# lucasnewman/f5-tts-mlx

Hardware: AMD Instinct MI355X
Metric: mel_frames_per_sec (higher is better)
Workload: dtype f16 (IEEE-half MFMA operands, fp32 accumulate / residual stream / LayerNorm / softmax state; meets the 1e-3 gate); 1 GPU; BASELINE configs[1]: F5-TTS 335M, 32-point euler (=62 DiT forwards, CFG), batch 1/GPU x 10 s (N=937) utterances, hipGraph=True; f16 (IEEE half) MFMA operands IN PLACE OF BASELINE's bf16 -- same width and MFMA rate, three more significand bits; plain bf16 fails the 1e-3 parity gate, see sub.b1_bf16; global_batch=1, seq_len=937, parallelism=dp1 (utterance sharding)

## Files before the change

### f5_tts_mlx_amd/csrc/convpos.hpp

```cpp
#include "op16.hpp"

#if F5_F16
#ifndef F5_CONVPOS_HPP_F16
#define F5_CONVPOS_HPP_F16
#define F5_CONVPOS_HPP_BODY
#endif
#else
#ifndef F5_CONVPOS_HPP_BF16
#define F5_CONVPOS_HPP_BF16
#define F5_CONVPOS_HPP_BODY
#endif
#endif
#ifdef F5_CONVPOS_HPP_BODY
#undef F5_CONVPOS_HPP_BODY
namespace F5_NS {

struct F5ConvPosArgs {
    const op16_t* in[2];
    const op16_t* W[2];
    const float* bias;
    int B, seq_len, C, groups, taps, ld;
    int nseg;
    int mode;
    op16_t* out_bf[2];
    float* out_f32;
    int ldo;
    int* sat_flag;
};

int f5_launch_convpos(const F5ConvPosArgs& a, hipStream_t stream);
}
#endif
```

### f5_tts_mlx_amd/csrc/engine.hip

```cpp
#include <stdarg.h>

#include <string>
#include <vector>

#include "../../include/f5tts_hip.h"
#include "host_common.hpp"

static Ops g_ops;

static thread_local char g_err[1024] = "";
void f5_set_error(const char* fmt, ...) {
    va_list ap;
    va_start(ap, fmt);
    vsnprintf(g_err, sizeof(g_err), fmt, ap);
    va_end(ap);
}
extern "C" const char* f5_last_error(void) { return g_err; }
extern "C" int f5_version(void) { return 1; }

struct MatF8 {
    size_t q = 0, s = 0;
    int rows = 0, ld = 0;
};
struct BlockW {
// ... 12 lines not shown
    size_t status;
    size_t lncnt, lncnt_words;
    size_t lens, dur2, text, ids, keep, rowkeep;
    size_t tgrid, dt, cfgv, sinus, th, temb, mod;
    size_t rope_cos, rope_sin;
    size_t rope_t;
    size_t cond, traj, ytmp, kst, vel;
    size_t xin[2];
    size_t te[2], tg, grn_partial, grn_nx;
    size_t tln[2], tg2[2], ct[2];
    size_t hc, x;
    size_t xb[2], c1[2], h[2], qk[2], vt[2], ao[2], ffh[2];
    size_t h8, h8s, ao8, ao8s, ffh8, ffh8s;
    size_t lnstats;
    size_t lnrowf;
    size_t lnmean;
    size_t foldc[2];
    bool fold_planned;
    size_t vt_bytes;
    size_t cond_keep;
};

struct F5Options {
    int q_premul = 1;
    int qkv_tr = 1;
    int fuse_ln = 0;
    int gemm_flags = 0;
    int attn_pipe = -1;
    int ln_fold = -1;
    int fold_stats = -1;
    int graph_split = 0;
    int sat_check = 1;
    int null_keeps_cond = 0;
};
static F5Options g_default_options;
static int g_live_engines = 0;
static int g_knob_epoch = 0;

struct f5_engine : WeightStore {
    f5_config cfg;
    int prec;
    size_t time_w0, time_b0, time_w2, time_b2;
    size_t ada_w, ada_b;
    size_t text_table, text_pos;
    std::vector<TextBlockW> tblocks;
    MatBF wx, wct;
    size_t bproj;
    MatBF conv_w[2];
    size_t conv_b[2];
    std::vector<BlockW> blocks;
    MatBF wout;
    size_t bout;
    Ops ops;
    F5Options opt = g_default_options;
    GraphCache graphs;
    std::vector<std::string> seen;
};

static int nfe_per_step(int method) { return method == F5_EULER ? 1 : (method == F5_MIDPOINT ? 2 : 4); }

static MatF8 alloc_f8(Bump& b, int rows, int ld) {
    MatF8 m;
    m.rows = rows;
    m.ld = ld;
    const int rows_pad = (rows + 255) / 256 * 256;
    m.q = b.take((size_t)rows_pad * ld);
// ... 123 lines not shown
    e->cfg = c;
    e->prec = precision;
    e->np = precision == F5_PREC_BF16X3 ? 2 : 1;
    e->f16 = e->ops.h = precision == F5_PREC_F16;
    build_arena_plan(e);
    ++g_live_engines;
    *out = e;
    return 0;
}

extern "C" void f5_engine_destroy(f5_engine* e) {
    if (!e) return;
    --g_live_engines;
    delete e;
}

extern "C" int f5_engine_set_graph_cache(f5_engine* e, int max_graphs) {
    F5_REQUIRE(e && max_graphs >= 1 && max_graphs <= 1024, "graph cache size must be in [1, 1024]");
    e->graphs.set_cap((size_t)max_graphs);
    return 0;
}

enum OptKind { OPT_SWITCH, OPT_TRI, OPT_INT };
static const struct OptDesc {
    const char* name;
    int F5Options::*member;
    OptKind kind;
} k_options[] = {
    {"q_premul", &F5Options::q_premul, OPT_SWITCH},     {"qkv_transposed", &F5Options::qkv_tr, OPT_SWITCH},
    {"ln_fusion", &F5Options::fuse_ln, OPT_SWITCH},     {"gemm_flags", &F5Options::gemm_flags, OPT_INT},
    {"attn_pipe", &F5Options::attn_pipe, OPT_TRI},      {"null_keeps_cond", &F5Options::null_keeps_cond, OPT_SWITCH},
    {"ln_fold", &F5Options::ln_fold, OPT_TRI},          {"sat_check", &F5Options::sat_check, OPT_SWITCH},
    {"graph_split", &F5Options::graph_split, OPT_SWITCH}, {"fold_stats", &F5Options::fold_stats, OPT_TRI},
};
static const OptDesc* find_option(const char* name) {
    std::string names;
    for (const OptDesc& o : k_options) {
        if (strcmp(o.name, name) == 0) return &o;
        names += names.empty() ? "" : ", ";
        names += o.name;
    }
    f5_set_error("unknown engine option %s (%s)", name, names.c_str());
    return nullptr;
}
extern "C" int f5_engine_set_option(f5_engine* e, const char* name, int value) {
    F5_REQUIRE(e && name, "null argument");
    const OptDesc* o = find_option(name);
    if (!o) return 2;
    e->opt.*o->member = o->kind == OPT_INT ? value : (o->kind == OPT_TRI && value < 0 ? -1 : (value ? 1 : 0));
    return 0;
}
extern "C" int f5_engine_get_option(f5_engine* e, const char* name, int* value) {
    F5_REQUIRE(e && name && value, "null argument");
    const OptDesc* o = find_option(name);
    if (!o) return 2;
    *value = e->opt.*o->member;
    return 0;
}
extern "C" int f5_engine_graph_count(f5_engine* e) { return e ? e->graphs.size() : -1; }

extern "C" int f5_weights_bytes(f5_engine* e, size_t* bytes) {
    F5_REQUIRE(e && bytes, "null argument");
    *bytes = e->arena_need;
    return 0;
}

extern "C" int f5_set_weights_arena(f5_engine* e, void* dev_arena, size_t bytes, void* stream) {
    F5_REQUIRE(e && dev_arena, "null argument");
    return e->set_arena(dev_arena, bytes, (hipStream_t)stream);
}

extern "C" int f5_load_tensor(f5_engine* e, const char* name, const float* host, int ndim, const int64_t* shape) {
    F5_REQUIRE(e && name && host && shape, "null argument");
    std::vector<TensorDst>* dsts = nullptr;
    size_t count = 0;
// ... 273 lines not shown
    int cur = 0;
    for (int i = 0; i < cf.conv_layers; ++i) {
        const TextBlockW& t = e->tblocks[i];
        RC(K.dwconv_ln(c.p<float>(w.te[cur]), c.a<float>(t.dw_w), c.a<float>(t.dw_b), c.a<float>(t.ln_w),
                               c.a<float>(t.ln_b), c.pb(w.tln, 0), c.pb(w.tln, 1), 2 * c.B, c.N, Dt, 1e-6f, s));
        F5GemmArgs g1 = gemm_base(c, c.pb(w.tln, 0), c.pb(w.tln, 1), Dt, t.pw1, M2, TF, Dt, c.a<float>(t.b1));
        g1.out_f32 = c.p<float>(w.tg);
        g1.ldo = TF;
        RC(K.gemm(g1, EPI_GELU_ERF, s));
        RC(K.grn(c.p<float>(w.tg), c.a<float>(t.gamma), c.a<float>(t.beta), c.p<float>(w.grn_partial),
                         c.p<float>(w.grn_nx), c.pb(w.tg2, 0), c.pb(w.tg2, 1), 2 * c.B, c.N, TF, s));
        F5GemmArgs g2 = gemm_base(c, c.pb(w.tg2, 0), c.pb(w.tg2, 1), TF, t.pw2, M2, Dt, TF, c.a<float>(t.b2));
        g2.out_f32 = c.p<float>(w.te[cur ^ 1]);
        g2.ldo = Dt;
        g2.resid = c.p<float>(w.te[cur]);
        g2.ldres = Dt;
        g2.rowkeep = c.p<uint8_t>(w.keep);
        RC(K.gemm(g2, EPI_RESID_KEEP, s));
        cur ^= 1;
    }
    if (c.edit)
        RC(K.pack_cond_text_keep(c.p<float>(w.cond), c.p<uint8_t>(w.cond_keep), c.p<float>(w.te[cur]), c.pb(w.ct, 0), c.pb(w.ct, 1),
                                 c.B, c.N, cf.mel_dim, Dt, e->opt.null_keeps_cond, s));
    else
        RC(K.pack_cond_text(c.p<float>(w.cond), c.p<int>(w.lens), c.p<float>(w.te[cur]), c.pb(w.ct, 0), c.pb(w.ct, 1), c.B,
                                c.N, cf.mel_dim, Dt, e->opt.null_keeps_cond, s));
    F5GemmArgs gh = gemm_base(c, c.pb(w.ct, 0), c.pb(w.ct, 1), 128 + Dt, e->wct, M2, D, 128 + Dt, c.a<float>(e->bproj));
    gh.out_f32 = c.p<float>(w.hc);
    gh.ldo = D;
    RC(K.gemm(gh, EPI_F32, s));
    return 0;
}

static int run_dit(const Ctx& c, int j) {
    const f5_engine* e = c.e;
    const f5_config& cf = e->cfg;
    const Workspace& w = c.w;
    const int D = cf.dim, FF = cf.ff_dim, L = cf.depth, H = cf.heads;
    const int M1 = c.B * c.N, M = c.nb * M1;
    hipStream_t s = c.s;
    const Ops& K = c.ops;
    const float* mod = c.p<float>(w.mod) + (size_t)j * (6 * L + 2) * D;
    const uint8_t* rowkeep = c.use_mask ? c.p<uint8_t>(w.rowkeep) : nullptr;
    const int* kvlen = c.use_mask ? c.p<int>(w.dur2) : nullptr;

    F5GemmArgs g0 = gemm_base(c, c.pb(w.xin, 0), c.pb(w.xin, 1), 128, e->wx, M, D, 128, nullptr);
    g0.a_row_mod = M1;
    g0.addrows = c.p<float>(w.hc);
    g0.ldadd = D;
    g0.out_f32 = c.p<float>(w.x);
    g0.ldo = D;
    g0.out_bf[0] = c.pb(w.xb, 0);
    g0.out_bf[1] = c.pb(w.xb, 1);
    g0.ldob = D;
    RC(K.gemm(g0, EPI_ADDROWS, s));

    F5ConvPosArgs cp;
    memset(&cp, 0, sizeof(cp));
    cp.B = c.nb * c.B;
    cp.seq_len = c.N;
    cp.C = D;
    cp.groups = cf.conv_pos_groups;
    cp.taps = cf.conv_pos_kernel;
    cp.ld = D;
    cp.ldo = D;
    cp.nseg = c.nseg();
    cp.in[0] = c.pb(w.xb, 0);
    cp.in[1] = c.pb(w.xb, 1);
    cp.W[0] = c.wm(e->conv_w[0], 0);
    cp.W[1] = c.wm(e->conv_w[0], 1);
    cp.bias = c.a<float>(e->conv_b[0]);
    cp.mode = 0;
    cp.out_bf[0] = c.pb(w.c1, 0);
    cp.out_bf[1] = c.pb(w.c1, 1);
    RC(K.convpos(cp, s));
    cp.in[0] = c.pb(w.c1, 0);
    cp.in[1] = c.pb(w.c1, 1);
    cp.W[0] = c.wm(e->conv_w[1], 0);
    cp.W[1] = c.wm(e->conv_w[1], 1);
    cp.bias = c.a<float>(e->conv_b[1]);
    cp.mode = 1;
    cp.out_bf[0] = cp.out_bf[1] = nullptr;
    cp.out_f32 = c.p<float>(w.x);
    RC(K.convpos(cp, s));

    const float qpre = q_premul_factor(e);
    for (int i = 0; i < L && e->prec == F5_PREC_MXFP8; ++i) {
        const BlockW& bw = e->blocks[i];
        const float* m6 = mod + (size_t)i * 6 * D;
        auto f8args = [&](const uint8_t* a8, const uint8_t* as, int lda, const MatF8& wm, int N_, int K_, const float* bias) {
            F5GemmArgs g;
            memset(&g, 0, sizeof(g));
            g.A8 = a8;
            g.As = as;
            g.lda8 = lda;
            g.W8 = (const uint8_t*)(e->arena + wm.q);
            g.Ws = (const uint8_t*)(e->arena + wm.s);
            g.ldw8 = wm.ld;
            g.M = M;
            g.N = N_;
            g.K = K_;
            g.nseg = 1;
            g.bias = bias;
            g.debug_flags = e->opt.gemm_flags;
            return g;
        };
        RC(f5_launch_ln_modulate_f8(c.p<float>(w.x), m6 + D, m6, c.p<uint8_t>(w.h8), c.p<uint8_t>(w.h8s), M, D, 1e-6f, s));
        F5GemmArgs gq = f8args(c.p<uint8_t>(w.h8), c.p<uint8_t>(w.h8s), D, bw.qkv8, 3 * D, D, c.a<float>(bw.bqkv));
        gq.out_bf[0] = c.pb(w.qk, 0);
        gq.ldob = 2 * D;
        gq.rope_cos = c.p<float>(w.rope_cos);
        gq.rope_sin = c.p<float>(w.rope_sin);
        gq.seq_len = c.N;
        gq.npad = c.npad;
        gq.heads = H;
        gq.dmodel = D;
        gq.vt[0] = c.pb(w.vt, 0);
// ... 959 lines not shown
extern "C" int f5_op_gemm_resid_gate_ln(const void* a_hi, const void* a_lo, const void* w_hi, const void* w_lo, const float* bias,
                                        const float* gate, const uint8_t* rowkeep, float* x, const float* ln_scale,
                                        const float* ln_shift, void* h_hi, void* h_lo, int* counters, int M, int N, int K, int lda,
                                        int ldw, int nseg, void* stream) {
    F5GemmArgs g = f5_gemm_args(a_hi, a_lo, w_hi, w_lo, lda, ldw, M, N, K, nseg, bias);
    g.gate = gate;
    g.rowkeep = rowkeep;
    g.out_f32 = x;
    g.ldo = N;
    g.ln_counter = counters;
    g.ln_scale = ln_scale;
    g.ln_shift = ln_shift;
    g.ln_out[0] = (op16_t*)h_hi;
    g.ln_out[1] = (op16_t*)h_lo;
    g.ln_eps = 1e-6f;
    F5_REQUIRE(gate && x && ln_scale && ln_shift && h_hi && counters, "gemm_resid_gate_ln: null pointer");
    return g_ops.gemm(g, EPI_RESID_GATE, (hipStream_t)stream);
}
extern "C" int f5_op_gemm_addrows(const void* a_hi, const void* a_lo, const void* w_hi, const void* w_lo, const float* addrows,
                                  int a_row_mod, float* out_f32, void* out_hi, void* out_lo, int M, int N, int K, int lda, int ldw,
                                  int ldo, int nseg, void* stream) {
    F5GemmArgs g = f5_gemm_args(a_hi, a_lo, w_hi, w_lo, lda, ldw, M, N, K, nseg, nullptr);
    g.a_row_mod = a_row_mod;
    g.addrows = addrows;
    g.ldadd = ldo;
    g.out_f32 = out_f32;
    g.ldo = ldo;
    g.out_bf[0] = (op16_t*)out_hi;
    g.out_bf[1] = (op16_t*)out_lo;
    g.ldob = ldo;
    F5_REQUIRE(addrows != nullptr && out_f32 != nullptr && out_hi != nullptr, "gemm_addrows: null addrows / out");
    return g_ops.gemm(g, EPI_ADDROWS, (hipStream_t)stream);
}
extern "C" int f5_op_layernorm(const float* x, const float* w, const float* b, float* out_f32, void* out_hi, void* out_lo,
                               int rows, int dim, void* stream) {
    return g_ops.layernorm(x, w, b, out_f32, (op16_t*)out_hi, (op16_t*)out_lo, rows, dim, 1e-6f, (hipStream_t)stream);
}
extern "C" int f5_op_im2col7(const float* x, void* out_hi, void* out_lo, int nbatch, int seq_len, int channels, void* stream) {
    return g_ops.im2col7(x, (op16_t*)out_hi, (op16_t*)out_lo, nbatch, seq_len, channels, (hipStream_t)stream);
}
extern "C" int f5_op_im2col7_ragged(const float* x, void* out_hi, void* out_lo, int nbatch, int seq_len, int channels,
                                    const int32_t* lens_dev, void* stream) {
    return g_ops.im2col7_ragged(x, (op16_t*)out_hi, (op16_t*)out_lo, nbatch, seq_len, channels, lens_dev, (hipStream_t)stream);
}
```

### f5_tts_mlx_amd/csrc/host_common.hpp

```cpp
#pragma once
#include <string>
#include <unordered_map>
#include <vector>

#define F5_F16 0
#include "attention.hpp"
#include "convpos.hpp"
#include "gemm.hpp"
#include "rowops.hpp"
#undef F5_F16
#define F5_F16 1
#include "attention.hpp"
#include "convpos.hpp"
#include "gemm.hpp"
#include "rowops.hpp"
#undef F5_F16

typedef f5bf::op16_t op16_t;
using f5bf::F5AttnArgs;
using f5bf::F5ConvPosArgs;
using f5bf::F5GemmArgs;
using f5bf::F5OdeArgs;
using f5bf::f5_grn_partial_floats;
using f5bf::f5_launch_duration_head;
using f5bf::f5_launch_gemm_f8;
using f5bf::f5_launch_ln_modulate_f8;
using f5bf::f5_launch_quantize_mx;
using f5bf::f5_launch_quantize_mx_bf16;
using f5bf::f5_launch_rope_table;
using f5bf::f5_launch_rope_table_g4;
using f5bf::f5_launch_rowkeep;
using f5bf::f5_launch_seconds_to_frames;
using f5bf::f5_launch_stage_words;
using f5bf::f5_launch_copy_words;
using f5bf::f5_launch_skinny_gemm;
using f5bf::f5_launch_splice;
using f5bf::f5_launch_splice_keep;
using f5bf::f5_launch_gather_frames;
using f5bf::f5_launch_copy_bytes;
using f5bf::f5_launch_text_embed;
using f5bf::f5_launch_text_pos_table;
using f5bf::f5_launch_time_sinus;

static inline F5GemmArgs f5_gemm_args(const void* a_hi, const void* a_lo, const void* w_hi, const void* w_lo, int lda, int ldw, int M, int N,
                                      int K, int nseg, const float* bias) {
    F5GemmArgs g;
    memset(&g, 0, sizeof(g));
    g.A[0] = (const op16_t*)a_hi;
    g.A[1] = (const op16_t*)a_lo;
    g.W[0] = (const op16_t*)w_hi;
    g.W[1] = (const op16_t*)w_lo;
    g.lda = lda;
    g.ldw = ldw;
// ... 1 lines not shown
    g.N = N;
    g.K = K;
    g.nseg = nseg;
    g.bias = bias;
    return g;
}

struct Ops {
    bool h = false;
    static f5hf::op16_t* H(op16_t* p) { return reinterpret_cast<f5hf::op16_t*>(p); }
    int gemm(const F5GemmArgs& a, int epi, hipStream_t s) const {
        return h ? f5hf::f5_launch_gemm(reinterpret_cast<const f5hf::F5GemmArgs&>(a), epi, s) : f5bf::f5_launch_gemm(a, epi, s);
    }
    int fold_rows(const float* stats, int ld, int nslice, int M, float eps, float* rowf, float* row_shift, hipStream_t s) const {
        return h ? f5hf::f5_launch_fold_rows(stats, ld, nslice, M, eps, rowf, row_shift, s)
                 : f5bf::f5_launch_fold_rows(stats, ld, nslice, M, eps, rowf, row_shift, s);
    }
    int fold_consts(const op16_t* w, int ldw, const float* bias, const float* scale, const float* shift, size_t vec_stride, int nvec, float* c1,
                    float* c2, size_t out_stride, int N, int K, hipStream_t s, int count = 1, size_t w_stride = 0, size_t bias_stride = 0,
                    size_t mod_stride = 0, size_t out_blk_stride = 0) const {
        if (h) {
            const f5hf::F5FoldBatch bt = {count, w_stride, bias_stride, mod_stride, out_blk_stride};
            return f5hf::f5_launch_fold_consts(reinterpret_cast<const f5hf::op16_t*>(w), ldw, bias, scale, shift, vec_stride, nvec, c1, c2,
                                               out_stride, N, K, s, &bt);
        }
        const f5bf::F5FoldBatch bt = {count, w_stride, bias_stride, mod_stride, out_blk_stride};
        return f5bf::f5_launch_fold_consts(w, ldw, bias, scale, shift, vec_stride, nvec, c1, c2, out_stride, N, K, s, &bt);
    }
    int attention(const F5AttnArgs& a, hipStream_t s) const {
        return h ? f5hf::f5_launch_attention(reinterpret_cast<const f5hf::F5AttnArgs&>(a), s) : f5bf::f5_launch_attention(a, s);
    }
    int convpos(const F5ConvPosArgs& a, hipStream_t s) const {
        return h ? f5hf::f5_launch_convpos(reinterpret_cast<const f5hf::F5ConvPosArgs&>(a), s) : f5bf::f5_launch_convpos(a, s);
    }
    int ode_stage(const F5OdeArgs& a, hipStream_t s) const {
        return h ? f5hf::f5_launch_ode_stage(reinterpret_cast<const f5hf::F5OdeArgs&>(a), s) : f5bf::f5_launch_ode_stage(a, s);
    }
    int ln_modulate(const float* x, const float* scale, const float* shift, op16_t* hi, op16_t* lo, int rows, int dim, float eps,
                    hipStream_t s, float* mean_out = nullptr) const {
        return h ? f5hf::f5_launch_ln_modulate(x, scale, shift, H(hi), H(lo), rows, dim, eps, s, mean_out)
                 : f5bf::f5_launch_ln_modulate(x, scale, shift, hi, lo, rows, dim, eps, s, mean_out);
    }
    int dwconv_ln(const float* x, const float* dw_w, const float* dw_b, const float* ln_w, const float* ln_b, op16_t* hi, op16_t* lo,
                  int nbatch, int seq_len, int dim, float eps, hipStream_t s) const {
        return h ? f5hf::f5_launch_dwconv_ln(x, dw_w, dw_b, ln_w, ln_b, H(hi), H(lo), nbatch, seq_len, dim, eps, s)
                 : f5bf::f5_launch_dwconv_ln(x, dw_w, dw_b, ln_w, ln_b, hi, lo, nbatch, seq_len, dim, eps, s);
    }
    int dwconv_ln_ragged(const float* x, const float* dw_w, const float* dw_b, const float* ln_w, const float* ln_b, op16_t* hi,
                         op16_t* lo, int nbatch, int seq_len, int dim, float eps, const int* lens, hipStream_t s) const {
        return h ? f5hf::f5_launch_dwconv_ln_ragged(x, dw_w, dw_b, ln_w, ln_b, H(hi), H(lo), nbatch, seq_len, dim, eps, lens, s)
                 : f5bf::f5_launch_dwconv_ln_ragged(x, dw_w, dw_b, ln_w, ln_b, hi, lo, nbatch, seq_len, dim, eps, lens, s);
    }
    int grn(const float* g, const float* gamma, const float* beta, float* partial, float* nx, op16_t* hi, op16_t* lo, int nbatch,
            int seq_len, int dim, hipStream_t s) const {
        return h ? f5hf::f5_launch_grn(g, gamma, beta, partial, nx, H(hi), H(lo), nbatch, seq_len, dim, s)
                 : f5bf::f5_launch_grn(g, gamma, beta, partial, nx, hi, lo, nbatch, seq_len, dim, s);
    }
    int pack_cond_text(const float* cond, const int* lens, const float* text_emb, op16_t* hi, op16_t* lo, int B, int seq_len,
                       int mel_dim, int dt, int null_keeps_cond, hipStream_t s) const {
        return h ? f5hf::f5_launch_pack_cond_text(cond, lens, text_emb, H(hi), H(lo), B, seq_len, mel_dim, dt, null_keeps_cond, s)
                 : f5bf::f5_launch_pack_cond_text(cond, lens, text_emb, hi, lo, B, seq_len, mel_dim, dt, null_keeps_cond, s);
    }
    int pack_cond_text_keep(const float* cond, const uint8_t* keep, const float* text_emb, op16_t* hi, op16_t* lo, int B, int seq_len,
                            int mel_dim, int dt, int null_keeps_cond, hipStream_t s) const {
        return h ? f5hf::f5_launch_pack_cond_text_keep(cond, keep, text_emb, H(hi), H(lo), B, seq_len, mel_dim, dt, null_keeps_cond, s)
                 : f5bf::f5_launch_pack_cond_text_keep(cond, keep, text_emb, hi, lo, B, seq_len, mel_dim, dt, null_keeps_cond, s);
// ... 328 lines not shown
```

### f5_tts_mlx_amd/engine.py

```python
from __future__ import annotations

import ctypes as C
import os
import warnings
from concurrent.futures import ThreadPoolExecutor
from pathlib import Path
from typing import Dict, Optional, Sequence

import numpy as np
import torch

from .weights import DiTConfig, check_weights

_LIB_PATH = Path(os.environ["F5TTS_HIP_LIB"]).resolve() if os.environ.get("F5TTS_HIP_LIB") else Path(__file__).resolve().parent / "csrc" / "libf5tts_hip.so"
_lib = None

METHODS = {"euler": 0, "midpoint": 1, "rk4": 2}
PRECISIONS = {"bf16": 0, "bf16x3": 1, "mxfp8": 2, "f16": 3}
GRAPH_MODES = {False: 0, True: 1, "off": 0, "on": 1, "auto": 2}


def operand_dtype(precision: str) -> torch.dtype:
    return torch.float16 if precision == "f16" else torch.bfloat16

# ... 89 lines not shown
    device = torch.device(device)
    y0 = torch.empty((B, int(N), int(mel)), dtype=torch.float32, device=device)
    CH = 256
    scratch = torch.empty(3 * min(B, CH), dtype=torch.int32, device=device)
    with torch.cuda.device(device):
        for b0 in range(0, B, CH):
            nb = min(CH, B - b0)
            c_seeds = (C.c_uint64 * nb)(*[int(s) & 0xFFFFFFFFFFFFFFFF for s in seeds[b0:b0 + nb]])
            c_durs = (C.c_int32 * nb)(*[int(d) for d in durations[b0:b0 + nb]])
            check(lib.f5_noise_normal(c_seeds, nb, c_durs, int(N), int(mel), ptr(y0[b0:b0 + nb]), ptr(scratch), stream_ptr(device)),
                  "f5_noise_normal")
    return y0


def to_c_config(cfg: DiTConfig) -> F5Config:
    return F5Config(cfg.dim, cfg.depth, cfg.heads, cfg.dim_head, cfg.ff_dim, cfg.mel_dim, cfg.text_num_embeds, cfg.text_dim,
                    cfg.text_ff_dim, cfg.conv_layers, cfg.conv_pos_kernel, cfg.conv_pos_groups, cfg.freq_embed_dim,
                    cfg.text_max_pos, int(bool(getattr(cfg, "text_mask_padding", True))))


def _aligned_bytes(nbytes: int, device: torch.device) -> torch.Tensor:
    t = torch.empty(int(nbytes) + 256, dtype=torch.uint8, device=device)
    off = (-t.data_ptr()) % 256
    return t[off:off + int(nbytes)]


class OperandRangeWarning(RuntimeWarning):
    """A 16-bit MFMA operand left the fp16 range in a call: the folded LayerNorm operand (the engine fell back to the unfolded path) or
    any other producer (the engine fell back to precision bf16x3)."""


RANGE_CHECKS = ("sync", "auto", "async", "off")
OPTION_NAMES = ("q_premul", "qkv_transposed", "ln_fusion", "gemm_flags", "attn_pipe", "null_keeps_cond", "ln_fold", "sat_check",
                "graph_split", "fold_stats")
SPLIT_MIN_BATCH = 0
STATUS_FOLD_OVERFLOW, STATUS_FOLD_RAN, STATUS_SATURATED = 1, 2, 4


class Engine:

    def __init__(self, cfg: DiTConfig, precision: str = "bf16", device: str | torch.device = "cuda:0", range_check: str = "sync",
                 keep_host_weights: bool = True, share_weights_with: Optional["Engine"] = None):
        if range_check not in RANGE_CHECKS:
            raise ValueError(f"range_check must be one of {RANGE_CHECKS}")
        if precision not in PRECISIONS:
            raise ValueError(f"unknown precision {precision!r}; expected one of {sorted(PRECISIONS)}")
        self.lib = load_library()
        self.cfg = cfg
        self.precision = precision
        self.device = torch.device(device)
        if self.device.type != "cuda":
            raise RuntimeError("the HIP engine needs a GPU device (cuda:N); there is no CPU path")
        torch.cuda.set_device(self.device)
        self._h = C.c_void_p()
        ccfg = to_c_config(cfg)
        check(self.lib.f5_engine_create(C.byref(ccfg), PRECISIONS[precision], C.byref(self._h)), "f5_engine_create")
        nbytes = C.c_size_t()
        check(self.lib.f5_weights_bytes(self._h, C.byref(nbytes)), "f5_weights_bytes")
        if share_weights_with is None:
            self.arena = _aligned_bytes(nbytes.value, self.device)
            check(self.lib.f5_set_weights_arena(self._h, ptr(self.arena), C.c_size_t(self.arena.numel()), stream_ptr(self.device)),
                  "f5_set_weights_arena")
        else:
            check(self.lib.f5_share_weights(self._h, share_weights_with._h), "f5_share_weights")
            self.arena = share_weights_with.arena
        self._workspace: Optional[torch.Tensor] = None
        self.weights_ready = share_weights_with is not None
# ... 395 lines not shown
```

### include/f5tts_hip.h

```cpp
#ifndef F5TTS_HIP_H
#define F5TTS_HIP_H

#include <stddef.h>
#include <stdint.h>

#ifdef __cplusplus
extern "C" {
#endif

typedef struct f5_engine f5_engine;

typedef struct f5_config {
    int32_t dim;
    int32_t depth;
    int32_t heads;
    int32_t dim_head;
    int32_t ff_dim;
    int32_t mel_dim;
    int32_t text_num_embeds;
    int32_t text_dim;
    int32_t text_ff_dim;
    int32_t conv_layers;
    int32_t conv_pos_kernel;
    int32_t conv_pos_groups;
// ... 102 lines not shown
                      int silu_out, void* stream);
int f5_op_cfg_axpy(const float* pred, const float* null_pred, float cfg, const float* base, const float* dt_dev, float coef,
                   float divisor, float* out, void* xin_hi, void* xin_lo, int rows, int mel_dim, void* stream);
int f5_op_ode_stage(const float* pred, const float* null_pred, float cfg, const float* cfg_ptr, const float* base, const float* dt_dev,
                    float coef, float divisor, int mode, float* kstore, const float* k1, const float* k2, const float* k3, float* out,
                    void* xin_hi, void* xin_lo, int rows, int mel_dim, void* stream);
int f5_op_pack_cond_text(const float* cond, const int32_t* lens, const float* text_emb, void* out_hi, void* out_lo, int B, int seq_len,
                         int mel_dim, int dt, int null_keeps_cond, void* stream);
int f5_op_pack_x(const float* y, void* out_hi, void* out_lo, int rows, int mel_dim, void* stream);
int f5_op_splice(const float* cond, const float* y, const int32_t* lens, float* out, int B, int seq_len, int mel_dim, void* stream);
int f5_op_pack_cond_text_keep(const float* cond, const uint8_t* keep, const float* text_emb, void* out_hi, void* out_lo, int B,
                              int seq_len, int mel_dim, int dt, int null_keeps_cond, void* stream);
int f5_op_splice_keep(const float* cond, const float* y, const uint8_t* keep, float* out, int B, int seq_len, int mel_dim, void* stream);
int f5_op_gather_frames(const float* src, const int32_t* src_idx, float* cond_out, uint8_t* keep_out, int B, int n_src, int seq_len,
                        int mel_dim, void* stream);
int f5_op_rowkeep(const int32_t* dur, uint8_t* keep, int nbatch, int seq_len, void* stream);
int f5_op_copy_words(const void* src, void* dst, size_t nwords, void* stream);
int f5_op_stage_words(const uint32_t* host_words, size_t nwords, uint32_t* dst, void* stream);
int f5_op_zero_vt_pad(void* vt, size_t rows, int seq_len, int npad, void* stream);

int f5_noise_normal(const uint64_t* seeds, int B, const int32_t* durations, int N, int mel, float* y0, void* scratch_words,
                    void* stream);
int f5_op_noise_from_bits(const uint32_t* bits_dev, size_t n, float* out, void* stream);

int f5_op_gemm_resid_gate(const void* a_hi, const void* a_lo, const void* w_hi, const void* w_lo, const float* bias,
                          const float* gate, const uint8_t* rowkeep, float* x, int M, int N, int K, int lda, int ldw, int ldx,
                          int nseg, void* stream);
int f5_op_gemm_resid_gate_ln(const void* a_hi, const void* a_lo, const void* w_hi, const void* w_lo, const float* bias,
                             const float* gate, const uint8_t* rowkeep, float* x, const float* ln_scale, const float* ln_shift,
                             void* h_hi, void* h_lo, int* counters, int M, int N, int K, int lda, int ldw, int nseg, void* stream);
int f5_op_gemm_addrows(const void* a_hi, const void* a_lo, const void* w_hi, const void* w_lo, const float* addrows,
                       int a_row_mod, float* out_f32, void* out_hi, void* out_lo, int M, int N, int K, int lda, int ldw, int ldo,
                       int nseg, void* stream);
int f5_op_layernorm(const float* x, const float* w, const float* b, float* out_f32, void* out_hi, void* out_lo, int rows,
                    int dim, void* stream);
int f5_op_im2col7(const float* x, void* out_hi, void* out_lo, int nbatch, int seq_len, int channels, void* stream);
int f5_op_istft(const float* x, int ldx, const float* window, float* frames_scratch, float* wave, int nframes, int n_fft,
                int hop, void* stream);

uint16_t f5_debug_f2h_bits(float f);
float f5_debug_h_bits2f(uint16_t h);
uint16_t f5_debug_f2bf_bits(float f);
int f5_debug_set_gemm_tile(int sel);
int f5_debug_last_gemm_kernel(char* buf, int n);
int f5_debug_last_attn_kernel(char* buf, int n);
int f5_debug_last_convpos_kernel(char* buf, int n);
int f5_debug_gemm_route(int epi, int M, int N, int nseg, int seq_len, int variant_bits, int debug_flags, char* name, int n, int* facts);
int f5_debug_set_gemm_flags(int v);
int f5_debug_set_gemm_order(int v);
int f5_debug_set_gemm_ring(int v);
int f5_debug_set_gemm_qkv_tile(int sel);
int f5_debug_set_gemm_nband(int n);
int f5_debug_set_convpos_tps(int taps);
int f5_debug_set_convpos_xcd_map(int on);
int f5_debug_set_attn_wide(int v);
int f5_debug_set_attn_kvsplit(int v);
int f5_debug_set_attn_pipe(int v);
int f5_debug_set_ln_fusion(int on);
int f5_debug_set_qkv_transposed(int on);
int f5_debug_set_q_premul(int on);
int f5_debug_set_op_fold_producer(const float* next_scale, void* x16_out, float* stats_out, const float* row_shift);
int f5_op_fold_rows(const float* stats, int nslice, int M, float* rowf, float* row_shift, void* stream);
int f5_debug_set_op_ln_mean_out(float* mean_out);
int f5_debug_set_op_fold_consumer(const float* rowf, const float* c1, const float* c2);
int f5_debug_set_op_fold_stats(const float* stats, int ld, const float* shift, float* mean_out);
int f5_debug_set_op_sat_flag(int* flag);
int f5_debug_set_op_fold_overflow_flag(int* flag);
int f5_op_fold_consts(const void* w_hi, int ldw, const float* bias, const float* scale, const float* shift, size_t vec_stride, int nvec,
                      float* c1, float* c2, size_t out_stride, int N, int K, void* stream);
int f5_debug_set_op_rope_tables_g4(const float* tq, const float* tk);
int f5_debug_set_op_q_premul(float factor);

int f5_op_quantize_mx(const float* x, int ldx, void* q, int ldq, void* scales, int rows, int cols, void* stream);
int f5_op_gemm_f8(const void* a8, const void* a_scales, const void* w8, const void* w_scales, const float* bias,
                  const float* gate, const uint8_t* rowkeep, float* out_f32, void* out_bf, void* out8, void* out8_scales,
                  int M, int N, int K, int lda8, int ldw8, int ldo, int epi, void* stream);

int f5_mel_spectrogram_batch(const float* wave, int B, int64_t L, const float* window, const float* filterbank, int n_fft, int hop,
                             int n_mels, float* out, void* stream);
// ... 86 lines not shown
```

Measured before the change: 13660 mel-frames/s.

## Fuse input projection and both conv-position layers into one kernel

Adds a fused front kernel that computes the input projection plus conditioning add, then both grouped conv-position layers with Mish, keeping intermediates in LDS and streaming conv weights through a multi-stage ring. It is chosen automatically when the workgroup count is small and precision is single-pass f16/bf16. It removes two launches and the global round trips of the projected activations and conv1 output, at the cost of recomputing a halo of projected rows per tile and lower parallelism per launch.

```diff
diff --git a/f5_tts_mlx_amd/csrc/convpos.hpp b/f5_tts_mlx_amd/csrc/convpos.hpp
--- a/f5_tts_mlx_amd/csrc/convpos.hpp
+++ b/f5_tts_mlx_amd/csrc/convpos.hpp
@@ -29,5 +29,26 @@
 };
 
 int f5_launch_convpos(const F5ConvPosArgs& a, hipStream_t stream);
+
+struct F5FrontArgs {
+    const op16_t* xin;
+    const op16_t* Wx;
+    const float* hc;
+    const op16_t* W1;
+    const op16_t* W2;
+    const float* b1;
+    const float* b2;
+    float* out;
+    int B, seq_len, C, groups, taps;
+    int kproj, lda, ldw, ldadd, ldo;
+    int a_row_mod;
+    int nseg;
+    int gemm_flags;
+    int ksplit;
+    int* sat_flag;
+};
+const char* f5_front_fused_refused(const F5FrontArgs& a);
+bool f5_front_fused_auto(const F5FrontArgs& a);
+int f5_launch_front_fused(const F5FrontArgs& a, hipStream_t stream);
 }
 #endif
diff --git a/f5_tts_mlx_amd/csrc/engine.hip b/f5_tts_mlx_amd/csrc/engine.hip
--- a/f5_tts_mlx_amd/csrc/engine.hip
+++ b/f5_tts_mlx_amd/csrc/engine.hip
@@ -68,6 +68,7 @@
     int graph_split = 0;
     int sat_check = 1;
     int null_keeps_cond = 0;
+    int front_fused = -1;
 };
 static F5Options g_default_options;
 static int g_live_engines = 0;
@@ -257,15 +258,19 @@
     {"attn_pipe", &F5Options::attn_pipe, OPT_TRI},      {"null_keeps_cond", &F5Options::null_keeps_cond, OPT_SWITCH},
     {"ln_fold", &F5Options::ln_fold, OPT_TRI},          {"sat_check", &F5Options::sat_check, OPT_SWITCH},
     {"graph_split", &F5Options::graph_split, OPT_SWITCH}, {"fold_stats", &F5Options::fold_stats, OPT_TRI},
+    {"front_fused", &F5Options::front_fused, OPT_TRI},
 };
+static const int k_options_listed = 10;
 static const OptDesc* find_option(const char* name) {
-    std::string names;
+    std::string names, later;
+    int i = 0;
     for (const OptDesc& o : k_options) {
         if (strcmp(o.name, name) == 0) return &o;
-        names += names.empty() ? "" : ", ";
-        names += o.name;
-    }
-    f5_set_error("unknown engine option %s (%s)", name, names.c_str());
+        std::string& dst = i++ < k_options_listed ? names : later;
+        dst += dst.empty() ? "" : ", ";
+        dst += o.name;
+    }
+    f5_set_error("unknown engine option %s (%s); also %s", name, names.c_str(), later.c_str());
     return nullptr;
 }
 extern "C" int f5_engine_set_option(f5_engine* e, const char* name, int value) {
@@ -605,17 +610,52 @@
     return 0;
 }
 
-static int run_dit(const Ctx& c, int j) {
+static int front_fused_choice(const F5FrontArgs& fa, bool one_pass_prec, int option) {
+    if (option == 0) return 0;
+    const char* why = one_pass_prec ? f5bf::f5_front_fused_refused(fa) : "f16 / bf16 precision only";
+    if (why != nullptr) {
+        if (option < 0) return 0;
+        f5_set_error("front_fused = 1: this shape / precision cannot run the fused front (%s)", why);
+        return -1;
+    }
+    return option == 1 || f5bf::f5_front_fused_auto(fa) ? 1 : 0;
+}
+
+static int run_dit_front(const Ctx& c) {
     const f5_engine* e = c.e;
     const f5_config& cf = e->cfg;
     const Workspace& w = c.w;
-    const int D = cf.dim, FF = cf.ff_dim, L = cf.depth, H = cf.heads;
+    const int D = cf.dim;
     const int M1 = c.B * c.N, M = c.nb * M1;
     hipStream_t s = c.s;
     const Ops& K = c.ops;
-    const float* mod = c.p<float>(w.mod) + (size_t)j * (6 * L + 2) * D;
-    const uint8_t* rowkeep = c.use_mask ? c.p<uint8_t>(w.rowkeep) : nullptr;
-    const int* kvlen = c.use_mask ? c.p<int>(w.dur2) : nullptr;
+
+    F5FrontArgs fa;
+    memset(&fa, 0, sizeof(fa));
+    fa.xin = c.pb(w.xin, 0);
+    fa.Wx = c.wm(e->wx, 0);
+    fa.hc = c.p<float>(w.hc);
+    fa.W1 = c.wm(e->conv_w[0], 0);
+    fa.W2 = c.wm(e->conv_w[1], 0);
+    fa.b1 = c.a<float>(e->conv_b[0]);
+    fa.b2 = c.a<float>(e->conv_b[1]);
+    fa.out = c.p<float>(w.x);
+    fa.B = c.nb * c.B;
+    fa.seq_len = c.N;
+    fa.C = D;
+    fa.groups = cf.conv_pos_groups;
+    fa.taps = cf.conv_pos_kernel;
+    fa.kproj = 128;
+    fa.lda = 128;
+    fa.ldw = e->wx.ld;
+    fa.ldadd = D;
+    fa.ldo = D;
+    fa.a_row_mod = M1;
+    fa.nseg = c.nseg();
+    fa.gemm_flags = e->opt.gemm_flags;
+    const int fused = front_fused_choice(fa, e->prec == F5_PREC_F16 || e->prec == F5_PREC_BF16, e->opt.front_fused);
+    if (fused < 0) return 2;
+    if (fused) return K.front_fused(fa, s);
 
     F5GemmArgs g0 = gemm_base(c, c.pb(w.xin, 0), c.pb(w.xin, 1), 128, e->wx, M, D, 128, nullptr);
     g0.a_row_mod = M1;
@@ -655,7 +695,22 @@
     cp.mode = 1;
     cp.out_bf[0] = cp.out_bf[1] = nullptr;
     cp.out_f32 = c.p<float>(w.x);
-    RC(K.convpos(cp, s));
+    return K.convpos(cp, s);
+}
+
+static int run_dit(const Ctx& c, int j) {
+    const f5_engine* e = c.e;
+    const f5_config& cf = e->cfg;
+    const Workspace& w = c.w;
+    const int D = cf.dim, FF = cf.ff_dim, L = cf.depth, H = cf.heads;
+    const int M1 = c.B * c.N, M = c.nb * M1;
+    hipStream_t s = c.s;
+    const Ops& K = c.ops;
+    const float* mod = c.p<float>(w.mod) + (size_t)j * (6 * L + 2) * D;
+    const uint8_t* rowkeep = c.use_mask ? c.p<uint8_t>(w.rowkeep) : nullptr;
+    const int* kvlen = c.use_mask ? c.p<int>(w.dur2) : nullptr;
+
+    RC(run_dit_front(c));
 
     const float qpre = q_premul_factor(e);
     for (int i = 0; i < L && e->prec == F5_PREC_MXFP8; ++i) {
@@ -1681,6 +1736,55 @@
     F5_REQUIRE(addrows != nullptr && out_f32 != nullptr && out_hi != nullptr, "gemm_addrows: null addrows / out");
     return g_ops.gemm(g, EPI_ADDROWS, (hipStream_t)stream);
 }
+extern "C" int f5_op_front_fused(const void* a_hi, const void* a_lo, const void* w_hi, const void* w_lo, const float* addrows, int a_row_mod,
+                                 float* out_f32, void* out_hi, void* out_lo, const void* conv1_w, const float* conv1_b, const void* conv2_w,
+                                 const float* conv2_b, int B, int seq_len, int C, int groups, int taps, int K, int lda, int ldw, int ldo,
+                                 int nseg, void* stream) {
+    (void)a_lo, (void)w_lo, (void)out_hi, (void)out_lo;
+    F5FrontArgs fa;
+    memset(&fa, 0, sizeof(fa));
+    fa.xin = (const op16_t*)a_hi;
+    fa.Wx = (const op16_t*)w_hi;
+    fa.hc = addrows;
+    fa.W1 = (const op16_t*)conv1_w;
+    fa.W2 = (const op16_t*)conv2_w;
+    fa.b1 = conv1_b;
+    fa.b2 = conv2_b;
+    fa.out = out_f32;
+    fa.B = B;
+    fa.seq_len = seq_len;
+    fa.C = C;
+    fa.groups = groups;
+    fa.taps = taps;
+    fa.kproj = K;
+    fa.lda = lda;
+    fa.ldw = ldw;
+    fa.ldadd = ldo;
+    fa.ldo = ldo;
+    fa.a_row_mod = a_row_mod;
+    fa.nseg = nseg;
+    return g_ops.front_fused(fa, (hipStream_t)stream);
+}
+extern "C" int f5_debug_front_fused_state(int B, int seq_len, int C, int groups, int taps, int K, int lda, int ldw, int nseg, int one_pass_prec,
+                                          int option, int* fused) {
+    F5_REQUIRE(fused != nullptr, "null argument");
+    F5FrontArgs fa;
+    memset(&fa, 0, sizeof(fa));
+    fa.B = B;
+    fa.seq_len = seq_len;
+    fa.C = C;
+    fa.groups = groups;
+    fa.taps = taps;
+    fa.kproj = K;
+    fa.lda = lda;
+    fa.ldw = ldw;
+    fa.ldadd = fa.ldo = C;
+    fa.nseg = nseg;
+    const int st = front_fused_choice(fa, one_pass_prec != 0, option < 0 ? -1 : (option ? 1 : 0));
+    if (st < 0) return 2;
+    *fused = st;
+    return 0;
+}
 extern "C" int f5_op_layernorm(const float* x, const float* w, const float* b, float* out_f32, void* out_hi, void* out_lo,
                                int rows, int dim, void* stream) {
     return g_ops.layernorm(x, w, b, out_f32, (op16_t*)out_hi, (op16_t*)out_lo, rows, dim, 1e-6f, (hipStream_t)stream);
diff --git a/f5_tts_mlx_amd/csrc/front.hip b/f5_tts_mlx_amd/csrc/front.hip
--- /dev/null
+++ b/f5_tts_mlx_amd/csrc/front.hip
@@ -0,0 +1,248 @@
+#include "convpos.hpp"
+#include "gemm_dev.hpp"
+#include "rowops.hpp"
+
+namespace F5_NS {
+extern int f5_gemm_debug_flags;
+extern int f5_convpos_xcd_map;
+
+#define FR_XLD 72
+#define FR_ROWS 128
+#define FR_MAXTAPS 31
+#define FR_KPROJ 128
+#define FR_XB_ROWS 192
+#define FR_C1_ROWS 160
+#define FR_NST 4
+constexpr int FR_SLAB = 64 * 64;
+constexpr int FR_XB_OFF = FR_NST * FR_SLAB;
+constexpr int FR_C1_OFF = FR_XB_OFF + FR_XB_ROWS * FR_XLD;
+constexpr int FR_E_OFF = FR_C1_OFF + FR_C1_ROWS * FR_XLD;
+constexpr int FR_SMEM = FR_E_OFF + FR_ROWS * 64 * 2;
+static_assert(FR_E_OFF % 8 == 0 && FR_SMEM * 2 <= 160 * 1024, "LDS layout");
+
+__global__ __launch_bounds__(512) void f5_front_fused_kernel(F5FrontArgs p) {
+    __shared__ __attribute__((aligned(16))) op16_t smem[FR_SMEM];
+    op16_t* const ring = smem;
+    op16_t* const sXb = smem + FR_XB_OFF;
+    op16_t* const sC1 = smem + FR_C1_OFF;
+    float* const sE = reinterpret_cast<float*>(smem + FR_E_OFF);
+
+    const int tid = threadIdx.x, lane = tid & 63;
+    const int wave = __builtin_amdgcn_readfirstlane(tid >> 6);
+    const int hi = lane >> 5, lr = lane & 31;
+    int n0, g, b;
+    int wg_rank, wg_count;
+    if (gridDim.y == 1 && (p.groups & 7) == 0) {
+        const int nx = (p.seq_len + FR_ROWS - 1) / FR_ROWS;
+        const int per_group = nx * p.B;
+        const int s_ = blockIdx.x >> 3;
+        const int gl = s_ / per_group, rem = s_ - gl * per_group;
+        g = gl * 8 + (blockIdx.x & 7);
+        b = rem / nx;
+        n0 = (rem - b * nx) * FR_ROWS;
+        wg_rank = rem;
+        wg_count = per_group;
+    } else {
+        n0 = blockIdx.x * FR_ROWS;
+        g = blockIdx.y;
+        b = blockIdx.z;
+        wg_rank = blockIdx.z * gridDim.x + blockIdx.x;
+        wg_count = gridDim.x * gridDim.z;
+    }
+    const int taps = p.taps, pad = taps >> 1, S = 2 * taps, kdim = taps * 64;
+    const int seq = p.seq_len;
+    const size_t rowbase = (size_t)b * seq;
+
+    const int wrow = tid >> 3;
+    const uint32_t wsrc = (uint32_t)((g * 64 + wrow) * kdim + (((tid & 7) ^ ((wrow >> 1) & 7)) << 3));
+#define FR_ISSUE(s_)                                                                            \
+    {                                                                                           \
+        const int ss_ = (s_);                                                                   \
+        const op16_t* W_ = ss_ < taps ? p.W1 : p.W2;                                            \
+        const int tap_ = ss_ < taps ? ss_ : ss_ - taps;                                         \
+        glds16(W_ + wsrc + tap_ * 64, ring + (ss_ & (FR_NST - 1)) * FR_SLAB + wave * 512);      \
+    }
+#pragma unroll
+    for (int st = 0; st < FR_NST - 1; ++st)
+        if (st < S) FR_ISSUE(st);
+
+    uint32_t warm = 0;
+    {
+        const int nlines = 2 * taps * 64;
+        int q = tid * wg_count + wg_rank;
+#pragma unroll 1
+        for (int i = 0; i < 8 && q < nlines; ++i, q += 512 * wg_count) {
+            const int sl = q >> 6, row = q & 63;
+            const op16_t* W_ = sl < taps ? p.W1 : p.W2;
+            warm ^= *reinterpret_cast<const uint32_t*>(W_ + (size_t)(g * 64 + row) * kdim + (sl < taps ? sl : sl - taps) * 64);
+        }
+    }
+
+    const int wv = wave & 1;
+    float b1v = p.b1[g * 64 + wv * 32 + lr], b2v = p.b2[g * 64 + wv * 32 + lr];
+    op16x8 ea[2][8], ew[2][8];
+    float ehc[2][16];
+#pragma unroll
+    for (int uu = 0; uu < 2; ++uu) {
+        const int u = wave + 8 * uu < 12 ? wave + 8 * uu : 11;
+        const int mb = u >> 1, nb = u & 1;
+        int n = n0 - 2 * pad + mb * 32 + lr;
+        n = n < 0 ? 0 : (n > seq - 1 ? seq - 1 : n);
+        size_t gr = rowbase + n;
+        if (p.a_row_mod > 0) gr = gr % (size_t)p.a_row_mod;
+        const op16_t* ap = p.xin + gr * p.lda + hi * 8;
+        const op16_t* wp = p.Wx + (size_t)(g * 64 + nb * 32 + lr) * p.ldw + hi * 8;
+#pragma unroll
+        for (int ks = 0; ks < 8; ++ks) {
+            ea[uu][ks] = *reinterpret_cast<const op16x8*>(ap + ks * 16);
+            ew[uu][ks] = *reinterpret_cast<const op16x8*>(wp + ks * 16);
+        }
+#pragma unroll
+        for (int r = 0; r < 16; ++r) {
+            int nn = n0 - 2 * pad + mb * 32 + (r & 3) + 8 * (r >> 2) + 4 * hi;
+            nn = nn < 0 ? 0 : (nn > seq - 1 ? seq - 1 : nn);
+            ehc[uu][r] = p.hc[(rowbase + nn) * p.ldadd + g * 64 + nb * 32 + lr];
+        }
+    }
+    f5_sat_t trk;
+    float zero = 0.0f;
+    asm volatile("" : "+v"(zero), "+v"(b1v), "+v"(b2v));
+    const bool ks2 = p.ksplit == 2;
+#pragma unroll
+    for (int uu = 0; uu < 2; ++uu) {
+        const int u = wave + 8 * uu < 12 ? wave + 8 * uu : 11;
+        const int mb = u >> 1, nb = u & 1;
+        f32x16 accA, accB;
+#pragma unroll
+        for (int e = 0; e < 16; ++e) accA[e] = 0.0f;
+#pragma unroll
+        for (int ks = 0; ks < 4; ++ks) accA = F5_MFMA32(ea[uu][ks], ew[uu][ks], accA, 0, 0, 0);
+#pragma unroll
+        for (int e = 0; e < 16; ++e) accB[e] = ks2 ? 0.0f : accA[e];
+#pragma unroll
+        for (int ks = 4; ks < 8; ++ks) accB = F5_MFMA32(ea[uu][ks], ew[uu][ks], accB, 0, 0, 0);
+#pragma unroll
+        for (int r = 0; r < 16; ++r) {
+            const int row = mb * 32 + (r & 3) + 8 * (r >> 2) + 4 * hi;
+            const int n = n0 - 2 * pad + row;
+            const bool ok = n >= 0 && n < seq;
+            float v = ks2 ? accA[r] + accB[r] : accB[r];
+            v = v + zero;
+            v += ehc[uu][r];
+            op16_t h = (op16_t)0.0f, l;
+            if (ok) f5_split(v, h, l, trk);
+            sXb[row * FR_XLD + nb * 32 + lr] = h;
+            const int cr = row - 2 * pad;
+            if (cr >= 0 && cr < FR_ROWS) sE[cr * 64 + nb * 32 + lr] = v;
+        }
+    }
+
+    const int mbw = wave >> 1;
+    const bool extra = wave < 2;
+    int woff[4];
+#pragma unroll
+    for (int ks = 0; ks < 4; ++ks) woff[ks] = swz_off(wv * 32 + lr, ks * 2 + hi);
+    const int aoff = (mbw * 32 + lr) * FR_XLD + hi * 8, aoffx = (128 + lr) * FR_XLD + hi * 8;
+    f32x16 acc, accx;
+#pragma unroll
+    for (int e = 0; e < 16; ++e) {
+        acc[e] = 0.0f;
+        accx[e] = 0.0f;
+    }
+    for (int s = 0; s < S; ++s) {
+        if (s + 2 < S) asm volatile("s_waitcnt vmcnt(2)" ::: "memory");
+        else asm volatile("s_waitcnt vmcnt(0)" ::: "memory");
+        asm volatile("s_waitcnt lgkmcnt(0)" ::: "memory");
+        __builtin_amdgcn_s_barrier();
+        asm volatile("" ::: "memory");
+        if (s + FR_NST - 1 < S) FR_ISSUE(s + FR_NST - 1);
+        const bool l1 = s < taps;
+        const int t = l1 ? s : s - taps;
+        const op16_t* src = (l1 ? sXb : sC1) + t * FR_XLD;
+        const op16_t* wsl = ring + (s & (FR_NST - 1)) * FR_SLAB;
+        op16x8 a[4], w[4], ax[4];
+#pragma unroll
+        for (int ks = 0; ks < 4; ++ks) {
+            a[ks] = *reinterpret_cast<const op16x8*>(src + aoff + ks * 16);
+            w[ks] = *reinterpret_cast<const op16x8*>(wsl + woff[ks]);
+            ax[ks] = a[ks];
+        }
+        if (l1 && extra) {
+#pragma unroll
+            for (int ks = 0; ks < 4; ++ks) ax[ks] = *reinterpret_cast<const op16x8*>(src + aoffx + ks * 16);
+        }
+#pragma unroll
+        for (int ks = 0; ks < 4; ++ks) acc = F5_MFMA32(a[ks], w[ks], acc, 0, 0, 0);
+        if (l1 && extra) {
+#pragma unroll
+            for (int ks = 0; ks < 4; ++ks) accx = F5_MFMA32(ax[ks], w[ks], accx, 0, 0, 0);
+        }
+        if (s == taps - 1) {
+#pragma unroll
+            for (int x = 0; x < 2; ++x) {
+                if (x == 1 && !extra) break;
+#pragma unroll
+                for (int r = 0; r < 16; ++r) {
+                    const int j = (x ? 128 : mbw * 32) + (r & 3) + 8 * (r >> 2) + 4 * hi;
+                    const int n = n0 - pad + j;
+                    op16_t h = (op16_t)0.0f, l;
+                    if (n >= 0 && n < seq) f5_split(f5_mish((x ? accx[r] : acc[r]) + b1v), h, l, trk);
+                    sC1[j * FR_XLD + wv * 32 + lr] = h;
+                }
+            }
+#pragma unroll
+            for (int e = 0; e < 16; ++e) acc[e] = 0.0f;
+        }
+    }
+#undef FR_ISSUE
+
+    float ev[16];
+#pragma unroll
+    for (int r = 0; r < 16; ++r) ev[r] = sE[(mbw * 32 + (r & 3) + 8 * (r >> 2) + 4 * hi) * 64 + wv * 32 + lr];
+#pragma unroll
+    for (int r = 0; r < 16; ++r) asm volatile("" : "+v"(ev[r]));
+#pragma unroll
+    for (int r = 0; r < 16; ++r) {
+        const int n = n0 + mbw * 32 + (r & 3) + 8 * (r >> 2) + 4 * hi;
+        if (n < seq) {
+            float m = f5_mish(acc[r] + b2v);
+            asm volatile("" : "+v"(m));
+            p.out[(rowbase + n) * p.ldo + g * 64 + wv * 32 + lr] = ev[r] + m;
+        }
+    }
+    f5_sat_commit(trk, p.sat_flag);
+}
+
+const char* f5_front_fused_refused(const F5FrontArgs& a) {
+    if (a.nseg != 1) return "single-segment operand modes only (f16 / bf16)";
+    if (a.B <= 0 || a.seq_len <= 0 || a.groups <= 0) return "bad shape";
+    if (a.C != a.groups * 64) return "channels per group must be 64";
+    if (a.taps < 1 || a.taps > FR_MAXTAPS || !(a.taps & 1)) return "taps must be odd and <= 31";
+    if (a.kproj != FR_KPROJ) return "the input projection must have K = 128";
+    if (a.lda % 8 != 0 || a.ldw % 8 != 0 || a.lda < FR_KPROJ || a.ldw < FR_KPROJ) return "lda / ldw must be multiples of 8 and >= 128";
+    if (a.ldadd < a.C || a.ldo < a.C) return "ldadd / ldo must be >= C";
+    return nullptr;
+}
+
+bool f5_front_fused_auto(const F5FrontArgs& a) {
+    const long nwg = (long)f5_cdiv(a.seq_len, FR_ROWS) * a.groups * a.B;
+    return nwg <= 256;
+}
+
+int f5_launch_front_fused(const F5FrontArgs& a, hipStream_t stream) {
+    const char* why = f5_front_fused_refused(a);
+    F5_REQUIRE(why == nullptr, "front_fused: %s", why);
+    F5_REQUIRE(a.xin && a.Wx && a.hc && a.W1 && a.W2 && a.b1 && a.b2 && a.out, "front_fused: null pointer");
+    dim3 grid(f5_cdiv(a.seq_len, FR_ROWS), a.groups, a.B);
+    const long nwg = (long)grid.x * grid.y * grid.z;
+    if (a.groups % 8 == 0 && f5_convpos_xcd_map) grid = dim3((unsigned)nwg, 1, 1);
+    F5FrontArgs ab = a;
+    if (ab.sat_flag == nullptr) ab.sat_flag = f5_sat_flag_host;
+    const F5GemmQuery q = {EPI_ADDROWS, a.B * a.seq_len, a.C, 1, 0, false, false, 0u, a.gemm_flags | f5_gemm_debug_flags};
+    const F5GemmKernel k = f5_gemm_route(q).kernel;
+    ab.ksplit = (k == F5K_RING_KS2_1 || k == F5K_RING_KS2_2) ? 2 : 1;
+    hipLaunchKernelGGL(f5_front_fused_kernel, grid, dim3(512), 0, stream, ab);
+    F5_LAUNCH_CHECK();
+    return 0;
+}
+}
diff --git a/f5_tts_mlx_amd/csrc/host_common.hpp b/f5_tts_mlx_amd/csrc/host_common.hpp
--- a/f5_tts_mlx_amd/csrc/host_common.hpp
+++ b/f5_tts_mlx_amd/csrc/host_common.hpp
@@ -19,6 +19,7 @@
 typedef f5bf::op16_t op16_t;
 using f5bf::F5AttnArgs;
 using f5bf::F5ConvPosArgs;
+using f5bf::F5FrontArgs;
 using f5bf::F5GemmArgs;
 using f5bf::F5OdeArgs;
 using f5bf::f5_grn_partial_floats;
@@ -86,6 +87,9 @@
     }
     int convpos(const F5ConvPosArgs& a, hipStream_t s) const {
         return h ? f5hf::f5_launch_convpos(reinterpret_cast<const f5hf::F5ConvPosArgs&>(a), s) : f5bf::f5_launch_convpos(a, s);
+    }
+    int front_fused(const F5FrontArgs& a, hipStream_t s) const {
+        return h ? f5hf::f5_launch_front_fused(reinterpret_cast<const f5hf::F5FrontArgs&>(a), s) : f5bf::f5_launch_front_fused(a, s);
     }
     int ode_stage(const F5OdeArgs& a, hipStream_t s) const {
         return h ? f5hf::f5_launch_ode_stage(reinterpret_cast<const f5hf::F5OdeArgs&>(a), s) : f5bf::f5_launch_ode_stage(a, s);
diff --git a/f5_tts_mlx_amd/engine.py b/f5_tts_mlx_amd/engine.py
--- a/f5_tts_mlx_amd/engine.py
+++ b/f5_tts_mlx_amd/engine.py
@@ -145,7 +145,7 @@
 
 RANGE_CHECKS = ("sync", "auto", "async", "off")
 OPTION_NAMES = ("q_premul", "qkv_transposed", "ln_fusion", "gemm_flags", "attn_pipe", "null_keeps_cond", "ln_fold", "sat_check",
-                "graph_split", "fold_stats")
+                "graph_split", "fold_stats", "front_fused")
 SPLIT_MIN_BATCH = 0
 STATUS_FOLD_OVERFLOW, STATUS_FOLD_RAN, STATUS_SATURATED = 1, 2, 4
 
diff --git a/include/f5tts_hip.h b/include/f5tts_hip.h
--- a/include/f5tts_hip.h
+++ b/include/f5tts_hip.h
@@ -158,6 +158,10 @@
 int f5_op_gemm_addrows(const void* a_hi, const void* a_lo, const void* w_hi, const void* w_lo, const float* addrows,
                        int a_row_mod, float* out_f32, void* out_hi, void* out_lo, int M, int N, int K, int lda, int ldw, int ldo,
                        int nseg, void* stream);
+int f5_op_front_fused(const void* a_hi, const void* a_lo, const void* w_hi, const void* w_lo, const float* addrows, int a_row_mod,
+                      float* out_f32, void* out_hi, void* out_lo, const void* conv1_w, const float* conv1_b, const void* conv2_w,
+                      const float* conv2_b, int B, int seq_len, int C, int groups, int taps, int K, int lda, int ldw, int ldo, int nseg,
+                      void* stream);
 int f5_op_layernorm(const float* x, const float* w, const float* b, float* out_f32, void* out_hi, void* out_lo, int rows,
                     int dim, void* stream);
 int f5_op_im2col7(const float* x, void* out_hi, void* out_lo, int nbatch, int seq_len, int channels, void* stream);
@@ -171,6 +175,8 @@
 int f5_debug_last_gemm_kernel(char* buf, int n);
 int f5_debug_last_attn_kernel(char* buf, int n);
 int f5_debug_last_convpos_kernel(char* buf, int n);
+int f5_debug_front_fused_state(int B, int seq_len, int C, int groups, int taps, int K, int lda, int ldw, int nseg, int one_pass_prec,
+                               int option, int* fused);
 int f5_debug_gemm_route(int epi, int M, int N, int nseg, int seq_len, int variant_bits, int debug_flags, char* name, int n, int* facts);
 int f5_debug_set_gemm_flags(int v);
 int f5_debug_set_gemm_order(int v);
```

Result: no change. 13790 mel-frames/s (median of 2 runs) (+1.0%).
